# yuanwu2017/llm-d

Hardware: AMD Instinct MI355X
Metric: output tok/s per decode GPU + p50 TTFT, Llama-3-70B P/D-disagg on 8×MI355X (higher is better)
Workload: dtype bf16; 1 GPU; model=Llama-3-70B, global_batch=64, seq_len=5000, isl=5000, osl=250, parallelism=dp1, block_size=64, graphs=True, kv_cache_dtype=auto, async_scheduling=True, setup_prompts_landed=63

## Files before the change

### llmd_amd/csrc/ops/bindings.cpp

```cpp
#include <torch/extension.h>
#include <c10/hip/HIPGuard.h>
#include <c10/hip/HIPStream.h>
#include <hip/hip_runtime.h>
#include <pybind11/stl.h>

#include <map>
#include <mutex>
#include <memory>
#include <vector>

extern "C" {
void llmd_rms_norm(void*, int64_t, const void*, int64_t, const void*, int, int, float, hipStream_t);
void llmd_layer_norm(void*, int64_t, void*, int64_t, void*, int64_t, const void*, const void*, int, int, float,
                     hipStream_t);
void llmd_fused_add_rms_norm(void*, int64_t, void*, int64_t, const void*, int, int, float,
                             hipStream_t);
int llmd_qk_rms_norm(void*, int64_t, const void*, const void*, int, int, int, int, float, hipStream_t);
void llmd_rope_cache(void*, int64_t, const int64_t*, const float*, int, int, int, int,
                     const int64_t*, void*, void*, int64_t, int, int, int, int, float, float, hipStream_t);
void llmd_gated_act(void*, int64_t, const void*, int64_t, int, int, int, float, float, hipStream_t);
int llmd_paged_decode(const void*, int64_t, const void*, const void*, int64_t, int, const int*, int,
                      const int*, int, int, int, int, float, int, const float*, int, int, void*,
                      int64_t, float*, float*, int, float, float, const int*, const int*, const int*,
                      const int*, int, int, int, const int*, hipStream_t);
// ... 28 lines not shown
                        hipStream_t);
int llmd_lora_bgmv(const void*, int64_t, const void*, const void*, int, int, int, int, const int*, float*, void*,
                   int64_t, hipStream_t);
int llmd_skinny_gemm(const void*, int64_t, const void*, int64_t, int, int, int, int, int, int, void*, int64_t,
                     float*, hipStream_t);
int llmd_dgemm_supported(int, int, int);
int llmd_mgemm(const void*, int64_t, const void*, int64_t, int, int, int, int, int, int, void*, int64_t, float*,
               int*, hipStream_t);
int llmd_mgemm_lds(int, int, int);
int llmd_mgemm_partials(const void*, int64_t, const void*, int64_t, int, int, int, int, int, int, float*, hipStream_t);
int llmd_reduce_rope_cache(const float*, int, int, void*, int64_t, const int64_t*, const float*, int, int, int, int,
                           const int64_t*, void*, void*, int64_t, int, int, int, int, float, float, hipStream_t);
int llmd_mgemm_add_rmsnorm(const void*, int64_t, const void*, int64_t, int, int, int, int, int, int, float*, void*,
                           int64_t, const void*, float, void*, int64_t, hipStream_t);
int llmd_mgemm_silu(const void*, int64_t, const void*, int64_t, int, int, int, int, int, void*, int64_t, hipStream_t);
int llmd_pgemm(const void*, int64_t, const void*, int64_t, void*, int64_t, int, int, int, int, int, void*,
               hipStream_t);
int64_t llmd_pgemm_ws_bytes(int, int, int, int, int);
int llmd_pgemm_fp8(const void*, int64_t, const float*, const void*, int64_t, const float*, void*, int64_t, int, int,
                   int, int, void*, hipStream_t);
int64_t llmd_pgemm_fp8_ws_bytes(int, int, int, int);
int llmd_mgemm_fp8(const void*, int64_t, const float*, const void*, int64_t, const float*, int, int, int, int, int,
                   int, void*, int64_t, float*, int*, hipStream_t);
int llmd_vmm_granularity(int, size_t*);
int llmd_vmm_alloc(int, size_t, int, void**, uint64_t*);
int llmd_vmm_export_fd(uint64_t, int*);
int llmd_vmm_import(const int*, int, size_t, int, void**, uint64_t*);
int llmd_vmm_free(void*, size_t, int, const uint64_t*);
int llmd_kvx_handle_size();
int llmd_kvx_dma_blocks(void*, const void*, int64_t, int64_t, const int*, int, int64_t, hipStream_t);
void llmd_moe_topk(const float*, int, int, int, int, const float*, int, int, int, float, int*, float*,
                   hipStream_t);
void llmd_moe_align(const int*, int, int, int, int*, int*, int*, int, int*, int*, hipStream_t);
// ... 428 lines not shown
  CHECK_CUDA(x); CHECK_BF16(x); CHECK_BF16(w); CHECK_BF16(out); CHECK_BF16(residual); CHECK_BF16(gamma);
  CHECK_INNER(x); CHECK_INNER(w); CHECK_INNER(out); CHECK_INNER(residual); CHECK_DT(part, at::kFloat);
  TORCH_CHECK(x.dim() == 2 && w.dim() == 2 && out.dim() == 2 && residual.dim() == 2, "mgemm_add_rmsnorm: 2-D operands");
  const int M = x.size(0), K = x.size(1), N = w.size(0);
  TORCH_CHECK(M >= 1 && M <= 128 && w.size(1) == K && K % 64 == 0 && N % 8 == 0, "mgemm_add_rmsnorm: shapes");
  TORCH_CHECK(out.size(0) == M && out.size(1) == N && residual.size(0) == M && residual.size(1) == N &&
              gamma.numel() == N, "mgemm_add_rmsnorm: output / residual / gamma shape");
  TORCH_CHECK(nsplit > 1 && part.numel() >= nsplit * (int64_t)M * N, "mgemm_add_rmsnorm: split-K workspace");
  int rc = llmd_mgemm_add_rmsnorm(x.data_ptr(), x.stride(0), w.data_ptr(), w.stride(0), M, N, K, (int)wrb,
                                  (int)nsplit, (int)stages, part.data_ptr<float>(), residual.data_ptr(),
                                  residual.stride(0), gamma.data_ptr(), (float)eps, out.data_ptr(), out.stride(0),
                                  cur_stream());
  TORCH_CHECK(rc == 0, "mgemm_add_rmsnorm failed: ", rc);
}

void pgemm(torch::Tensor y, torch::Tensor x, torch::Tensor w, int64_t epi, int64_t variant, bool split_k) {
  const c10::hip::OptionalHIPGuard device_guard(dev_of(y));
  CHECK_CUDA(x); CHECK_BF16(x); CHECK_BF16(w); CHECK_BF16(y); CHECK_INNER(x); CHECK_INNER(w); CHECK_INNER(y);
  TORCH_CHECK(x.dim() == 2 && w.dim() == 2 && y.dim() == 2, "pgemm: 2-D operands");
  const int64_t M = x.size(0), K = x.size(1), N = w.size(0);
  TORCH_CHECK(w.size(1) == K && K % 64 == 0 && N % 256 == 0, "pgemm: N % 256 == 0, K % 64 == 0");
  TORCH_CHECK(y.size(0) == M && y.size(1) == ((epi == 1 || epi == 3) ? N / 2 : N), "pgemm: output shape");
  TORCH_CHECK(epi != 3 || (variant >= 3 && variant <= 6), "pgemm: epi 3 (SiLU on the [gate; up] weight) needs variant 3-6");
  TORCH_CHECK(x.stride(0) % 8 == 0 && w.stride(0) % 8 == 0 && y.stride(0) % 8 == 0, "pgemm: 16-B row alignment");
  torch::Tensor ws;
  const int64_t wsb = split_k ? llmd_pgemm_ws_bytes((int)M, (int)N, (int)K, (int)epi, (int)variant) : 0;
  if (wsb > 0) ws = torch::empty({wsb / 4}, x.options().dtype(torch::kFloat));
  int rc = llmd_pgemm(x.data_ptr(), x.stride(0), w.data_ptr(), w.stride(0), y.data_ptr(), y.stride(0), (int)M,
                      (int)N, (int)K, (int)epi, (int)variant, wsb > 0 ? ws.data_ptr() : nullptr, cur_stream());
  TORCH_CHECK(rc == 0, "pgemm failed: ", rc);
}

void pgemm_fp8(torch::Tensor y, torch::Tensor xq, torch::Tensor xs, torch::Tensor wq, torch::Tensor ws, int64_t epi,
               bool split_k) {
  const c10::hip::OptionalHIPGuard device_guard(dev_of(y));
  CHECK_CUDA(xq); CHECK_BF16(y); CHECK_INNER(xq); CHECK_INNER(wq); CHECK_INNER(y);
  TORCH_CHECK(xq.scalar_type() == at::kFloat8_e4m3fn && wq.scalar_type() == at::kFloat8_e4m3fn, "pgemm_fp8: e4m3fn");
  TORCH_CHECK(xs.scalar_type() == at::kFloat && ws.scalar_type() == at::kFloat, "pgemm_fp8: fp32 scales");
  TORCH_CHECK(xs.is_contiguous() && ws.is_contiguous(), "pgemm_fp8: contiguous scales");
  TORCH_CHECK(xq.dim() == 2 && wq.dim() == 2 && y.dim() == 2, "pgemm_fp8: 2-D operands");
  const int64_t M = xq.size(0), K = xq.size(1), N = wq.size(0);
  TORCH_CHECK(wq.size(1) == K && K % 128 == 0 && N % 256 == 0, "pgemm_fp8: N % 256 == 0, K % 128 == 0");
  TORCH_CHECK(xs.numel() == M && ws.numel() == N, "pgemm_fp8: per-token / per-channel scales");
  TORCH_CHECK(epi == 0 || epi == 3, "pgemm_fp8: epi 0 or 3");
  TORCH_CHECK(y.size(0) == M && y.size(1) == (epi == 3 ? N / 2 : N), "pgemm_fp8: output shape");
// ... 740 lines not shown
  m.def("kvx_dma_blocks", &kvx_dma_blocks);
  m.def("kvx_ipc_export", &kvx_ipc_export);
  m.def("kvx_ipc_open", &kvx_ipc_open);
  m.def("kvx_ipc_close", &kvx_ipc_close);
  m.def("mla_attention", &mla_attention);
  m.def("mla_v2_shape", &mla_v2_shape, "H=128 MLA kernel shape: 10 * waves + head blocks per wave");
  m.def("skinny_gemm", &skinny_gemm);
  m.def("skinny_supported", &skinny_supported);
  m.def("mgemm", &mgemm);
  m.def("mgemm_partials", &mgemm_partials, "split-K partials of the medium-M GEMM (no reduce); returns nsplit");
  m.def("reduce_rope_cache", &reduce_rope_cache, "QKV split-K reduce + RoPE + paged cache write");
  m.def("mgemm_add_rmsnorm", &mgemm_add_rmsnorm, "decode o / down projection with residual-add + RMSNorm in its split-K reduce");
  m.def("pgemm_fp8", &pgemm_fp8, "prefill fp8 W8A8 GEMM (256x256 LDS-DMA tiles on 16x16x128 f8f6f4 MFMA), "
        "per-token x per-channel scales, optional fused SiLU-and-mul");
  m.def("pgemm", &pgemm, "prefill bf16 GEMM (256x256 LDS-DMA MFMA tiles), optional fused SiLU-and-mul",
        py::arg("y"), py::arg("x"), py::arg("w"), py::arg("epi"), py::arg("variant"), py::arg("split_k") = true);
  m.def("mgemm_fp8", &mgemm_fp8);
  m.def("mgemm_lds", [](int64_t M, int64_t wrb, int64_t stages) { return llmd_mgemm_lds((int)M, (int)wrb, (int)stages); });
  m.def("lora_bgmv", &lora_bgmv);
  m.def("mla_rope_cache", &mla_rope_cache);
  m.def("vmm_granularity", &vmm_granularity);
  m.def("vmm_pool", &vmm_pool);
  m.def("vmm_import", &vmm_import);
  m.def("vmm_release", &vmm_release);
  m.def("moe_topk", &moe_topk);
  m.def("moe_align", &moe_align, py::arg("ids"), py::arg("E"), py::arg("sorted_ids"), py::arg("tile_expert"),
        py::arg("expert_offsets"), py::arg("total_p"), py::arg("inv"), py::arg("tile_m") = 0);
  m.def("moe_gemm", &moe_gemm, py::arg("X"), py::arg("topk"), py::arg("sorted_ids"), py::arg("tile_expert"),
        py::arg("W"), py::arg("Y"), py::arg("mode"), py::arg("act"), py::arg("alpha"), py::arg("limit"),
        py::arg("a_rows_are_slots"), py::arg("bias"), py::arg("tile_m") = 0);
  m.def("moe_combine", &moe_combine);
// ... 33 lines not shown
```

### llmd_amd/csrc/ops/pgemm.hip

```cpp
#include <algorithm>
#include <type_traits>

#include "llmd_common.h"

using namespace llmd;

namespace {

constexpr int BM = 256, BN = 256, BK = 64, NT = 512;
constexpr int HALF = 16384;
constexpr int BUF = 4 * HALF;
constexpr int LDS_BYTES = 2 * BUF;
constexpr int GROUP_M = 8;

enum { EPI_NONE = 0, EPI_SILU = 1, EPI_F32 = 2, EPI_SILU_STD = 3 };

__device__ __forceinline__ void dma16(const void* src, char* lds) {
  __builtin_amdgcn_global_load_lds((const void __attribute__((address_space(1)))*)src,
                                   (void __attribute__((address_space(3)))*)lds, 16, 0, 0);
}

__device__ __forceinline__ void wait_vm(int n) {
  switch (n) {
    case 0: asm volatile("s_waitcnt vmcnt(0)" ::: "memory"); break;
// ... 774 lines not shown
#pragma unroll 4
    for (int it = 0; it < 16; ++it) {
      const int row = wc * 64 + it * 4 + (lane >> 4), c = lane & 15;
      const int m = m0 + wr * 128 + row;
      const int off = row * 256 + ((c ^ (row & 15)) * 16);
      float gf[8], uf[8], of[8];
      unpack8(*reinterpret_cast<const u32x4_t*>(gimg + off), gf);
      unpack8(*reinterpret_cast<const u32x4_t*>(uimg + off), uf);
#pragma unroll
      for (int e = 0; e < 8; ++e) of[e] = gf[e] / (1.f + __expf(-gf[e])) * uf[e];
      if (m < M) *reinterpret_cast<u32x4_t*>(C + (int64_t)m * ldc + n0 / 2 + c * 8) = pack8(of);
    }
  }
}

template <int EPI>
__global__ __launch_bounds__(NT6, 1) void pgemm7_kernel(const uint16_t* __restrict__ A, int64_t lda,
                                                        const uint16_t* __restrict__ W, int64_t ldw,
                                                        uint16_t* __restrict__ C, int64_t ldc, int M, int N, int K,
                                                        int ntiles) {
  constexpr int RB = 37;
  __shared__ __attribute__((aligned(1024))) char lds[2 * BUF6];
  const int tiles_m = (M + BM - 1) / BM, tiles_n = N / BN;
  const int P = gridDim.x;
  const int b = xcd_remap(blockIdx.x, P);
  const int nt = (ntiles - b + P - 1) / P;
  const int nk = K / BK;
  const int S = nt * nk;

  const int tid = threadIdx.x, lane = tid & 63;
// ... 197 lines not shown
__host__ inline void pgemm_plan(int M, int N, int K, int epi, int& full, int& tail, int& nsplit) {
  const int ntiles = ((M + BM - 1) / BM) * (N / BN), nk = K / BK;
  full = ntiles;
  tail = 0;
  nsplit = 1;
  const int t = ntiles % PG_CUS;
  if (epi != EPI_NONE || t == 0 || 2 * t > PG_CUS || nk < 32) return;
  int s = PG_CUS / t;
  s = std::min(s, nk / 8);
  if (s < 2) return;
  full = ntiles - t;
  tail = t;
  nsplit = s;
}

}

extern "C" int64_t llmd_pgemm_ws_bytes(int M, int N, int K, int epi, int variant) {
  if (M <= 0 || N % BN || K % BK) return 0;
  int full, tail, nsplit;
  pgemm_plan(M, N, K, epi, full, tail, nsplit);
  return nsplit > 1 ? (int64_t)nsplit * tail * BM * BN * 4 : 0;
}

extern "C" int llmd_pgemm(const void* A, int64_t lda, const void* W, int64_t ldw, void* C, int64_t ldc, int M, int N,
                          int K, int epi, int variant, void* ws, hipStream_t st) {
  if (M <= 0) return 0;
  if (N % BN || K % BK || lda % 8 || ldw % 8 || ldc % 8) return -1;
  if (epi == EPI_SILU_STD && (variant < 3 || variant > 6)) return -3;
  if ((int64_t)(M - 1) * lda + K > 0x7fffffffLL || (int64_t)(N - 1) * ldw + K > 0x7fffffffLL) return -2;
  const int ntiles = ((M + BM - 1) / BM) * (N / BN);
  if (variant == 6) {
    if (((int64_t)(M - 1) * lda + K) * 2 > 0x7fffffffLL || ((int64_t)(N - 1) * ldw + K) * 2 > 0x7fffffffLL) return -2;
    int full = ntiles, tail = 0, nsplit = 1;
    if (ws != nullptr) pgemm_plan(M, N, K, epi == EPI_SILU_STD ? EPI_SILU : epi, full, tail, nsplit);
    const auto* a = (const uint16_t*)A;
    const auto* w = (const uint16_t*)W;
    auto* c = (uint16_t*)C;
    const int P = std::min(full, PG_CUS);
    if (epi == EPI_SILU_STD)
      hipLaunchKernelGGL(pgemm7_kernel<EPI_SILU_STD>, dim3(P), dim3(NT6), 0, st, a, lda, w, ldw, c, ldc, M, N, K, full);
    else if (epi == EPI_NONE && full > 0)
      hipLaunchKernelGGL(pgemm7_kernel<EPI_NONE>, dim3(P), dim3(NT6), 0, st, a, lda, w, ldw, c, ldc, M, N, K, full);
    else if (epi != EPI_NONE)
      return -3;
    if (nsplit > 1) {
      hipLaunchKernelGGL((pgemm6_kernel<EPI_F32, 37, 0>), dim3(tail * nsplit), dim3(NT6), 0, st, a, lda, w, ldw, c, ldc,
                         M, N, K, full, nsplit, (float*)ws);
      hipLaunchKernelGGL(pgemm_splitk_reduce, dim3(tail * (BM / 8)), dim3(256), 0, st, (const float*)ws, nsplit,
                         tail, full, c, ldc, M, N);
    }
    return (int)hipGetLastError();
  }
  if (variant >= 3 && variant <= 5) {
    if (((int64_t)(M - 1) * lda + K) * 2 > 0x7fffffffLL || ((int64_t)(N - 1) * ldw + K) * 2 > 0x7fffffffLL) return -2;
    int full = ntiles, tail = 0, nsplit = 1;
    if (ws != nullptr) pgemm_plan(M, N, K, epi, full, tail, nsplit);
    const auto* a = (const uint16_t*)A;
    const auto* w = (const uint16_t*)W;
    auto* c = (uint16_t*)C;
    auto launch = [&](auto k_silu, auto k_std, auto k_none, auto k_f32) {
      if (epi == EPI_SILU)
        hipLaunchKernelGGL(k_silu, dim3(full), dim3(NT6), 0, st, a, lda, w, ldw, c, ldc, M, N, K, 0, 1, nullptr);
      else if (epi == EPI_SILU_STD)
        hipLaunchKernelGGL(k_std, dim3(full), dim3(NT6), 0, st, a, lda, w, ldw, c, ldc, M, N, K, 0, 1, nullptr);
      else if (full > 0)
        hipLaunchKernelGGL(k_none, dim3(full), dim3(NT6), 0, st, a, lda, w, ldw, c, ldc, M, N, K, 0, 1, nullptr);
      if (nsplit > 1) {
        hipLaunchKernelGGL(k_f32, dim3(tail * nsplit), dim3(NT6), 0, st, a, lda, w, ldw, c, ldc, M, N, K, full,
                           nsplit, (float*)ws);
        hipLaunchKernelGGL(pgemm_splitk_reduce, dim3(tail * (BM / 8)), dim3(256), 0, st, (const float*)ws, nsplit,
                           tail, full, c, ldc, M, N);
      }
    };
    if (variant == 3)
      launch(pgemm6_kernel<EPI_SILU, 37, 0>, pgemm6_kernel<EPI_SILU_STD, 37, 0>, pgemm6_kernel<EPI_NONE, 37, 0>,
             pgemm6_kernel<EPI_F32, 37, 0>);
    else if (variant == 4)
      launch(pgemm6_kernel<EPI_SILU, 37, 16>, pgemm6_kernel<EPI_SILU_STD, 37, 16>, pgemm6_kernel<EPI_NONE, 37, 16>,
             pgemm6_kernel<EPI_F32, 37, 16>);
    else
      launch(pgemm6_kernel<EPI_SILU, 44, 0>, pgemm6_kernel<EPI_SILU_STD, 44, 0>, pgemm6_kernel<EPI_NONE, 44, 0>,
// ... 63 lines not shown
```

### llmd_amd/models/llama.py

```python
from __future__ import annotations

from typing import Optional

import torch

from llmd_amd import ops
from llmd_amd.engine.attn_meta import AttnMeta
from llmd_amd.engine.config import ModelConfig
from llmd_amd.parallel.state import get_state

from .layers import ColumnLinear, LMHead, PagedAttention, RMSNorm, RowLinear, VocabEmbedding, wants_fp8_input


class LlamaMLP(torch.nn.Module):
    def __init__(self, cfg: ModelConfig, device):
        super().__init__()
        self.gate_up = ColumnLinear(cfg.hidden_size, 2 * cfg.intermediate_size, device=device)
        self.down = RowLinear(cfg.intermediate_size, cfg.hidden_size, device=device)

    def forward(self, x):
        return self.down(self.hidden(x))

    def hidden(self, x):
        gu = self.gate_up
        if (gu.lora is None and gu.bias is None and not wants_fp8_input(self.down) and x.dim() == 2
                and gu.weight.dtype == torch.bfloat16):
            v = ops.pgemm_silu_plan(x, gu.weight)
            if v is not None:
                return ops.pgemm_silu(x, gu.weight, variant=v)
            p = ops.mgemm_silu_plan(x, gu.weight)
            if p is not None:
                return ops.mgemm_silu(x, gu.weight, p)
        x0 = x[0] if isinstance(x, tuple) else x
        if (wants_fp8_input(self.down) and wants_fp8_input(gu) and gu.bias is None and x0.dim() == 2
                and ops._gpu(x0) and ops.pgemm8_silu_planned(x0.shape[0], gu.weight.shape[0], gu.weight.shape[1])):
            xq, xs = x if isinstance(x, tuple) else ops.quant_fp8_rows(x)
            if ops.pgemm_fp8_ok(xq, gu.weight):
                return ops.quant_fp8_rows(ops.pgemm_fp8(xq, xs, gu.weight, gu.weight_scale, epi=3))
        h = gu(x)
        if wants_fp8_input(self.down):
            return ops.gated_act_quant(h, ops.ACT_SILU)
        return ops.gated_act(h, ops.ACT_SILU)


# ... 172 lines not shown
```

### llmd_amd/ops/__init__.py

```python
from __future__ import annotations

import logging
import math
import os
from typing import Optional

import torch

from . import reference as ref

log = logging.getLogger("llmd.ops")

_C = None
_C_ERR: Exception | None = None


def native():
    global _C, _C_ERR
    if _C is not None:
        return _C
    import importlib

    debug = os.environ.get("LLMD_KERNEL_DEBUG", "0") == "1"
    name = "llmd_amd._C_debug" if debug else "llmd_amd._C"
# ... 1087 lines not shown


def mgemm_ok(x: torch.Tensor, w: torch.Tensor, max_m: int = 256) -> bool:
    M = x.shape[0] if x.dim() == 2 else -1
    return (_gpu(x) and 1 <= M <= max_m and x.shape[1] % 64 == 0 and x.dtype == torch.bfloat16
            and w.dtype == torch.bfloat16 and w.shape[0] % 4 == 0 and x.stride(-1) == 1 and x.stride(0) % 8 == 0
            and w.is_contiguous())


_MGEMM_MS = (64, 96, 128, 192, 256)


PGEMM_VARIANT = int(os.environ.get("LLMD_PGEMM_VARIANT", "0"))


def pgemm(x: torch.Tensor, w: torch.Tensor, epi: int = 0, out: Optional[torch.Tensor] = None,
          variant: Optional[int] = None, split_k: bool = True) -> torch.Tensor:
    M = x.shape[0]
    N = w.shape[0]
    if out is None:
        out = torch.empty(M, N // 2 if epi in (1, 3) else N, dtype=x.dtype, device=x.device)
    native().pgemm(out, x, w, epi, PGEMM_VARIANT if variant is None else variant, split_k)
    return out


def pgemm_silu(x: torch.Tensor, w: torch.Tensor, variant: int = 3, out: Optional[torch.Tensor] = None):
    return pgemm(x, w, epi=3, out=out, variant=variant, split_k=False)


def pgemm_pack_gate_up(w: torch.Tensor) -> torch.Tensor:
    F2, K = w.shape
    F = F2 // 2
    assert F % 128 == 0, F
    g = w[:F].view(F // 128, 128, K)
    u = w[F:].view(F // 128, 128, K)
    return torch.stack((g, u), 1).reshape(F2, K).contiguous()


def pgemm_ok(x: torch.Tensor, w: torch.Tensor) -> bool:
    return (x.dim() == 2 and x.dtype == torch.bfloat16 and w.dtype == torch.bfloat16 and x.is_cuda
            and w.shape[0] % 256 == 0 and w.shape[1] % 64 == 0 and x.stride(-1) == 1 and x.stride(0) % 8 == 0
            and w.is_contiguous())
# ... 13 lines not shown
PGEMM_MIN_M = int(os.environ.get("LLMD_PGEMM_MIN_M", "256"))
_pgemm_pick: dict = {}


def _time_ms(fn, reps: int = 2) -> float:
    fn()
    st, en = torch.cuda.Event(enable_timing=True), torch.cuda.Event(enable_timing=True)
    st.record()
    for _ in range(reps):
        fn()
    en.record()
    en.synchronize()
    return st.elapsed_time(en) / reps


def pgemm_plan(M: int, N: int, K: int) -> Optional[tuple[int, bool]]:
    from .pgemm_table import PGEMM_TABLE

    e = PGEMM_TABLE.get(((M + 255) // 256, N, K))
    return None if e is None else e[0]


def pgemm_silu_plan(x: torch.Tensor, w: torch.Tensor) -> Optional[int]:
    if PGEMM_AUTO == "0" or x.shape[0] < PGEMM_MIN_M or not pgemm_ok(x, w) or (w.shape[0] // 2) % 128:
        return None
    from .pgemm_table import PGEMM_TABLE

    e = PGEMM_TABLE.get(("silu", (x.shape[0] + 255) // 256, w.shape[0], w.shape[1]))
    return None if e is None or e[0] is None else e[0][0]


def pgemm_wins(x: torch.Tensor, w: torch.Tensor) -> Optional[tuple[int, bool]]:
    M, (N, K) = x.shape[0], w.shape
    if PGEMM_AUTO != "measure":
        return pgemm_plan(M, N, K)
    key = ((M + 255) // 256, N, K)
    c = _pgemm_pick.get(key, False)
    if c is False:
        if torch.cuda.is_current_stream_capturing():
            return None
        y = torch.empty(M, N, dtype=x.dtype, device=x.device)
        t_pg = _time_ms(lambda: pgemm(x, w, out=y))
        t_bl = _time_ms(lambda: torch.nn.functional.linear(x, w))
        c = _pgemm_pick[key] = (PGEMM_VARIANT, True) if t_pg < 0.97 * t_bl else None
        msg = (f"prefill GEMM M~{M} N={N} K={K}: pgemm {t_pg:.3f} ms, hipBLASLt {t_bl:.3f} ms -> "
               f"{'pgemm' if c else 'hipBLASLt'}")
        log.debug(msg)
        if os.environ.get("LLMD_PGEMM_VERBOSE") == "1":
            import sys

            print(msg, file=sys.stderr, flush=True)
    return c


def linear(x: torch.Tensor, w: torch.Tensor, bias: Optional[torch.Tensor] = None) -> torch.Tensor:
    if PGEMM_AUTO != "0" and x.dim() == 2 and x.shape[0] >= PGEMM_MIN_M and pgemm_ok(x, w):
        plan = pgemm_wins(x, w)
        if plan is not None:
            y = pgemm(x, w, variant=plan[0], split_k=plan[1])
            return y if bias is None else y.add_(bias)
    if _SKINNY:
        M = x.shape[0] if x.dim() == 2 else 0
        if 33 <= M <= 256 and mgemm_ok(x, w):
            plan = mgemm_choice(M, w.shape[0], w.shape[1])
            if plan is not None:
                y = mgemm(x, w, plan)
                return y if bias is None else y.add_(bias)
        if skinny_ok(x, w):
            plan = dgemm_choice(M, w.shape[0], w.shape[1])
            if plan is not None:
                y = skinny_gemm(x, w, plan)
                return y if bias is None else y.add_(bias)
    return torch.nn.functional.linear(x, w, bias)

# ... 3 lines not shown
```

### llmd_amd/ops/pgemm_table.py

```python

PGEMM_TABLE = {
    (2, 4096, 4096): (None, 35.5, 26.0),
    (3, 4096, 4096): (None, 38.8, 28.9),
    (4, 4096, 4096): (None, 44.9, 34.1),
    (6, 4096, 4096): (None, 57.2, 46.9),
    (8, 4096, 4096): (None, 67.2, 57.4),
    (12, 4096, 4096): (None, 78.7, 75.7),
    (16, 4096, 4096): (None, 92.9, 88.1),
    (18, 4096, 4096): ((3, True), 127.5, 141.3),
    (20, 4096, 4096): (None, 137.7, 135.1),
    (24, 4096, 4096): (None, 159.1, 153.9),
    (32, 4096, 4096): (None, 183.7, 175.9),
    (2, 4096, 14336): ((3, True), 65.4, 78.2),
    (3, 4096, 14336): ((3, True), 84.4, 93.0),
    (4, 4096, 14336): ((3, True), 101.4, 112.2),
    (6, 4096, 14336): (None, 152.1, 151.7),
    (8, 4096, 14336): ((3, True), 172.0, 182.4),
    (12, 4096, 14336): (None, 258.8, 246.9),
    (16, 4096, 14336): (None, 318.4, 290.9),
    (18, 4096, 14336): ((0, True), 405.5, 756.1),
    (20, 4096, 14336): (None, 455.5, 443.1),
    (24, 4096, 14336): (None, 528.7, 506.9),
    (32, 4096, 14336): (None, 678.8, 595.5),
    (2, 5120, 8192): ((3, True), 54.1, 57.0),
# ... 8 lines not shown
    (24, 5120, 8192): (None, 339.1, 328.3),
    (32, 5120, 8192): ((3, False), 486.1, 651.4),
    (2, 6144, 4096): (None, 40.4, 31.8),
    (3, 6144, 4096): (None, 47.3, 34.3),
    (4, 6144, 4096): (None, 56.4, 45.6),
    (6, 6144, 4096): (None, 71.4, 61.0),
    (8, 6144, 4096): (None, 77.7, 73.3),
    (12, 6144, 4096): ((3, True), 127.1, 138.1),
    (16, 6144, 4096): (None, 157.6, 151.7),
    (18, 6144, 4096): (None, 167.5, 165.3),
    (20, 6144, 4096): (None, 178.9, 174.3),
    (24, 6144, 4096): (None, 225.7, 227.6),
    (32, 6144, 4096): (None, 273.4, 264.5),
    (2, 8192, 4096): (None, 46.6, 35.9),
    (3, 8192, 4096): (None, 56.6, 42.0),
    (4, 8192, 4096): (None, 66.0, 55.9),
    (6, 8192, 4096): (None, 78.3, 75.4),
    (8, 8192, 4096): (None, 92.7, 88.8),
    (12, 8192, 4096): (None, 156.9, 150.5),
    (16, 8192, 4096): (None, 183.5, 177.8),
    (18, 8192, 4096): (None, 227.5, 226.9),
    (20, 8192, 4096): ((3, True), 248.7, 354.7),
    (24, 8192, 4096): (None, 275.3, 264.3),
    (32, 8192, 4096): (None, 365.5, 349.5),
    (2, 8192, 8192): (None, 69.3, 68.2),
    (3, 8192, 8192): (None, 92.9, 78.5),
    (4, 8192, 8192): (None, 107.0, 105.9),
    (6, 8192, 8192): (None, 148.4, 143.4),
    (8, 8192, 8192): (None, 174.9, 170.3),
    (12, 8192, 8192): (None, 301.9, 291.4),
    (16, 8192, 8192): (None, 350.5, 336.4),
    (18, 8192, 8192): (None, 436.4, 440.9),
    (20, 8192, 8192): ((3, False), 482.5, 667.5),
    (24, 8192, 8192): (None, 523.1, 506.2),
    (32, 8192, 8192): (None, 701.3, 675.2),
    (2, 8192, 14336): (None, 112.9, 116.2),
    (3, 8192, 14336): (None, 173.8, 143.9),
    (4, 8192, 14336): ((3, True), 192.9, 206.2),
    (6, 8192, 14336): (None, 267.5, 258.3),
    (8, 8192, 14336): (None, 325.4, 307.1),
    (12, 8192, 14336): (None, 523.5, 525.7),
    (16, 8192, 14336): (None, 630.5, 600.7),
    (18, 8192, 14336): (None, 781.4, 801.0),
    (20, 8192, 14336): ((3, True), 856.5, 1081.4),
    (24, 8192, 14336): (None, 1012.4, 909.5),
    (32, 8192, 14336): (None, 1342.3, 1210.8),
    (2, 8192, 28672): ((3, True), 212.5, 314.7),
    (3, 8192, 28672): (None, 335.0, 270.3),
    (4, 8192, 28672): (None, 364.2, 362.3),
    (6, 8192, 28672): (None, 583.4, 508.3),
    (8, 8192, 28672): (None, 653.8, 628.6),
    (12, 8192, 28672): ((3, True), 1004.7, 1044.5),
    (16, 8192, 28672): (None, 1316.1, 1238.6),
    (18, 8192, 28672): (None, 1549.3, 1591.1),
    (20, 8192, 28672): ((3, True), 1694.7, 2340.8),
    (24, 8192, 28672): (None, 1998.6, 1912.4),
    (32, 8192, 28672): (None, 2659.9, 2518.2),
    (2, 10240, 8192): (None, 81.1, 80.3),
    (3, 10240, 8192): (None, 102.3, 102.1),
    (4, 10240, 8192): (None, 135.7, 127.8),
    (6, 10240, 8192): (None, 167.0, 164.9),
    (8, 10240, 8192): ((3, True), 249.0, 263.2),
    (12, 10240, 8192): (None, 341.3, 325.5),
    (16, 10240, 8192): ((3, True), 466.9, 667.1),
    (18, 10240, 8192): (None, 529.0, 492.6),
    (20, 10240, 8192): ((3, True), 597.1, 665.1),
    (24, 10240, 8192): (None, 691.7, 659.0),
    (32, 10240, 8192): (None, 879.8, 853.7),
    (2, 28672, 4096): (None, 89.8, 88.7),
    ("silu", 2, 28672, 4096): ((6, False), 91.3, 103.9),
    (3, 28672, 4096): (None, 152.1, 134.0),
    ("silu", 3, 28672, 4096): (None, 163.8, 150.6),
    (4, 28672, 4096): (None, 178.2, 172.4),
    ("silu", 4, 28672, 4096): ((3, False), 182.7, 192.4),
    (6, 28672, 4096): (None, 262.4, 257.7),
    ("silu", 6, 28672, 4096): ((6, False), 272.9, 288.6),
    (8, 28672, 4096): (None, 353.9, 332.9),
    ("silu", 8, 28672, 4096): ((6, False), 362.4, 374.1),
    (12, 28672, 4096): (None, 516.7, 520.9),
    ("silu", 12, 28672, 4096): ((6, False), 537.0, 566.1),
    (16, 28672, 4096): (None, 648.9, 611.8),
    ("silu", 16, 28672, 4096): ((6, False), 669.8, 692.7),
    (18, 28672, 4096): (None, 746.3, 701.2),
    ("silu", 18, 28672, 4096): ((6, False), 755.3, 786.9),
    (20, 28672, 4096): ((3, True), 831.7, 893.4),
    ("silu", 20, 28672, 4096): ((3, False), 852.6, 976.0),
    (24, 28672, 4096): ((3, True), 1008.1, 1076.1),
    ("silu", 24, 28672, 4096): ((6, False), 1028.2, 1180.9),
    (32, 28672, 4096): (None, 1288.0, 1251.4),
    ("silu", 32, 28672, 4096): ((3, False), 1323.5, 1389.5),
    (2, 28672, 8192): (None, 197.6, 186.2),
    ("silu", 2, 28672, 8192): (None, 201.1, 200.1),
    (3, 28672, 8192): (None, 274.2, 261.6),
    ("silu", 3, 28672, 8192): (None, 318.8, 273.5),
    (4, 28672, 8192): (None, 347.3, 340.0),
    ("silu", 4, 28672, 8192): ((3, False), 355.7, 417.4),
    (6, 28672, 8192): (None, 511.5, 512.9),
    ("silu", 6, 28672, 8192): ((3, False), 526.5, 536.0),
    (8, 28672, 8192): (None, 660.7, 660.7),
    ("silu", 8, 28672, 8192): (None, 691.6, 687.8),
    (12, 28672, 8192): (None, 975.6, 974.7),
    ("silu", 12, 28672, 8192): (None, 1047.4, 1020.5),
    (16, 28672, 8192): (None, 1241.5, 1209.7),
    ("silu", 16, 28672, 8192): (None, 1278.9, 1270.3),
    (18, 28672, 8192): (None, 1511.8, 1412.0),
    ("silu", 18, 28672, 8192): (None, 1484.1, 1469.4),
    (20, 28672, 8192): ((3, False), 1601.0, 1652.6),
    ("silu", 20, 28672, 8192): ((3, False), 1636.7, 1722.6),
    (24, 28672, 8192): ((3, True), 1940.4, 2082.5),
    ("silu", 24, 28672, 8192): ((3, False), 1981.2, 2163.8),
    (32, 28672, 8192): (None, 2464.3, 2435.3),
    ("silu", 32, 28672, 8192): (None, 2552.3, 2566.0),
    (2, 57344, 8192): (None, 384.7, 371.3),
    ("silu", 2, 57344, 8192): (None, 393.1, 388.1),
    (3, 57344, 8192): (None, 528.2, 522.0),
# ... 21 lines not shown
```

Before: 383.3 output tok/s (whole job).

## Add half-height tail tiles to prefill GEMM to balance the last wave

Adds a new prefill GEMM tail mode that runs the leftover tiles of a partial wave as two 128-row half-tiles each, so more CUs stay busy when the tile count leaves a small remainder modulo the CU count. It plumbs a tail-form argument through the C ABI, bindings and Python wrappers, and adds a host-side plan query. The per-shape table is updated to select the half-tile form for several Llama-relevant shapes, including the gate_up SiLU path at some M buckets. Half tiles cost more weight traffic per output element and add a second kernel launch.

```diff
diff --git a/llmd_amd/csrc/ops/bindings.cpp b/llmd_amd/csrc/ops/bindings.cpp
--- a/llmd_amd/csrc/ops/bindings.cpp
+++ b/llmd_amd/csrc/ops/bindings.cpp
@@ -66,9 +66,10 @@
 int llmd_mgemm_add_rmsnorm(const void*, int64_t, const void*, int64_t, int, int, int, int, int, int, float*, void*,
                            int64_t, const void*, float, void*, int64_t, hipStream_t);
 int llmd_mgemm_silu(const void*, int64_t, const void*, int64_t, int, int, int, int, int, void*, int64_t, hipStream_t);
-int llmd_pgemm(const void*, int64_t, const void*, int64_t, void*, int64_t, int, int, int, int, int, void*,
+int llmd_pgemm(const void*, int64_t, const void*, int64_t, void*, int64_t, int, int, int, int, int, int, void*,
                hipStream_t);
-int64_t llmd_pgemm_ws_bytes(int, int, int, int, int);
+int64_t llmd_pgemm_ws_bytes(int, int, int, int, int, int);
+int llmd_pgemm_plan(int, int, int, int, int, int*, int*, int*);
 int llmd_pgemm_fp8(const void*, int64_t, const float*, const void*, int64_t, const float*, void*, int64_t, int, int,
                    int, int, void*, hipStream_t);
 int64_t llmd_pgemm_fp8_ws_bytes(int, int, int, int);
@@ -527,7 +528,7 @@
   TORCH_CHECK(rc == 0, "mgemm_add_rmsnorm failed: ", rc);
 }
 
-void pgemm(torch::Tensor y, torch::Tensor x, torch::Tensor w, int64_t epi, int64_t variant, bool split_k) {
+void pgemm(torch::Tensor y, torch::Tensor x, torch::Tensor w, int64_t epi, int64_t variant, int64_t tail) {
   const c10::hip::OptionalHIPGuard device_guard(dev_of(y));
   CHECK_CUDA(x); CHECK_BF16(x); CHECK_BF16(w); CHECK_BF16(y); CHECK_INNER(x); CHECK_INNER(w); CHECK_INNER(y);
   TORCH_CHECK(x.dim() == 2 && w.dim() == 2 && y.dim() == 2, "pgemm: 2-D operands");
@@ -537,11 +538,21 @@
   TORCH_CHECK(epi != 3 || (variant >= 3 && variant <= 6), "pgemm: epi 3 (SiLU on the [gate; up] weight) needs variant 3-6");
   TORCH_CHECK(x.stride(0) % 8 == 0 && w.stride(0) % 8 == 0 && y.stride(0) % 8 == 0, "pgemm: 16-B row alignment");
   torch::Tensor ws;
-  const int64_t wsb = split_k ? llmd_pgemm_ws_bytes((int)M, (int)N, (int)K, (int)epi, (int)variant) : 0;
+  TORCH_CHECK(tail >= 0 && tail <= 2, "pgemm: tail 0 (none), 1 (split-K) or 2 (half tiles)");
+  TORCH_CHECK(tail != 2 || variant == 3, "pgemm: the half-tile tail needs variant 3");
+  const int64_t wsb = llmd_pgemm_ws_bytes((int)M, (int)N, (int)K, (int)epi, (int)variant, (int)tail);
   if (wsb > 0) ws = torch::empty({wsb / 4}, x.options().dtype(torch::kFloat));
   int rc = llmd_pgemm(x.data_ptr(), x.stride(0), w.data_ptr(), w.stride(0), y.data_ptr(), y.stride(0), (int)M,
-                      (int)N, (int)K, (int)epi, (int)variant, wsb > 0 ? ws.data_ptr() : nullptr, cur_stream());
+                      (int)N, (int)K, (int)epi, (int)variant, (int)tail, wsb > 0 ? ws.data_ptr() : nullptr,
+                      cur_stream());
   TORCH_CHECK(rc == 0, "pgemm failed: ", rc);
+}
+
+std::tuple<int64_t, int64_t, int64_t, int64_t, int64_t> pgemm_plan(int64_t M, int64_t N, int64_t K, int64_t epi,
+                                                                   int64_t tail) {
+  int full = 0, t = 0, nsplit = 1;
+  const int form = llmd_pgemm_plan((int)M, (int)N, (int)K, (int)epi, (int)tail, &full, &t, &nsplit);
+  return {form, full, t, nsplit, llmd_pgemm_ws_bytes((int)M, (int)N, (int)K, (int)epi, 3, (int)tail)};
 }
 
 void pgemm_fp8(torch::Tensor y, torch::Tensor xq, torch::Tensor xs, torch::Tensor wq, torch::Tensor ws, int64_t epi,
@@ -1312,7 +1323,8 @@
   m.def("pgemm_fp8", &pgemm_fp8, "prefill fp8 W8A8 GEMM (256x256 LDS-DMA tiles on 16x16x128 f8f6f4 MFMA), "
         "per-token x per-channel scales, optional fused SiLU-and-mul");
   m.def("pgemm", &pgemm, "prefill bf16 GEMM (256x256 LDS-DMA MFMA tiles), optional fused SiLU-and-mul",
-        py::arg("y"), py::arg("x"), py::arg("w"), py::arg("epi"), py::arg("variant"), py::arg("split_k") = true);
+        py::arg("y"), py::arg("x"), py::arg("w"), py::arg("epi"), py::arg("variant"), py::arg("tail") = 1);
+  m.def("pgemm_plan", &pgemm_plan, "launch plan of the prefill GEMM under a tail form (host only)");
   m.def("mgemm_fp8", &mgemm_fp8);
   m.def("mgemm_lds", [](int64_t M, int64_t wrb, int64_t stages) { return llmd_mgemm_lds((int)M, (int)wrb, (int)stages); });
   m.def("lora_bgmv", &lora_bgmv);
diff --git a/llmd_amd/csrc/ops/pgemm.hip b/llmd_amd/csrc/ops/pgemm.hip
--- a/llmd_amd/csrc/ops/pgemm.hip
+++ b/llmd_amd/csrc/ops/pgemm.hip
@@ -812,6 +812,178 @@
   }
 }
 
+constexpr int HM = 128;
+constexpr int IMGH = 16384;
+
+template <int EPI>
+__global__ __launch_bounds__(NT6, 1) void pgemm6h_kernel(const uint16_t* __restrict__ A, int64_t lda,
+                                                         const uint16_t* __restrict__ W, int64_t ldw,
+                                                         uint16_t* __restrict__ C, int64_t ldc, int M, int N, int K,
+                                                         int tile0) {
+  static_assert(EPI == EPI_NONE || EPI == EPI_SILU_STD, "half tiles: no packed-SiLU or fp32-partial form");
+  __shared__ __attribute__((aligned(1024))) char lds[2 * BUF6];
+  const int tiles_m = (M + BM - 1) / BM, tiles_n = N / BN;
+  const int b = xcd_remap(blockIdx.x, gridDim.x);
+  const int nk = K / BK;
+  int tm, tn;
+  tile_mn(tile0 + (b >> 1), tiles_m, tiles_n, tm, tn);
+  const int m0 = tm * BM + (b & 1) * HM, n0 = tn * BN;
+  if (m0 >= M) return;
+
+  const int tid = threadIdx.x, lane = tid & 63;
+  const int w = __builtin_amdgcn_readfirstlane(tid >> 6);
+  const int wr = w >> 1, wc = w & 1;
+
+  const __amdgpu_buffer_rsrc_t ra = __builtin_amdgcn_make_buffer_rsrc((void*)A, 0, 0x7fffffff, 0x00020000);
+  const __amdgpu_buffer_rsrc_t rw = __builtin_amdgcn_make_buffer_rsrc((void*)W, 0, 0x7fffffff, 0x00020000);
+  uint32_t va[4], vw[8];
+#pragma unroll
+  for (int j = 0; j < 4; ++j) {
+    const int row = 32 * w + 8 * j + (lane >> 3);
+    const int c = (lane & 7) ^ ((row >> 1) & 7);
+    va[j] = m0 + row < M ? (uint32_t)(((m0 + row) * lda + c * 8) * 2) : 0x80000000u;
+  }
+#pragma unroll
+  for (int j = 0; j < 8; ++j) {
+    const int row = 64 * w + 8 * j + (lane >> 3);
+    const int c = (lane & 7) ^ ((row >> 1) & 7);
+    const int wrow = EPI == EPI_SILU_STD ? (row < 128 ? 0 : N / 2 - 128) + tn * 128 + row : n0 + row;
+    vw[j] = (uint32_t)((wrow * ldw + c * 8) * 2);
+  }
+  auto dma_a = [&](int kt, int j) {
+    const uint32_t so = (uint32_t)(min(kt, nk - 1) * BK * 2);
+    char* dst = lds + (kt & 1) * BUF6 + (4 * w + j) * 1024;
+    __builtin_amdgcn_raw_ptr_buffer_load_lds(ra, (__attribute__((address_space(3))) void*)dst, 16, va[j], so, 0, 0);
+  };
+  auto dma_w = [&](int kt, int j) {
+    const uint32_t so = (uint32_t)(min(kt, nk - 1) * BK * 2);
+    char* dst = lds + (kt & 1) * BUF6 + OPB6 + (8 * w + j) * 1024;
+    __builtin_amdgcn_raw_ptr_buffer_load_lds(rw, (__attribute__((address_space(3))) void*)dst, 16, vw[j], so, 0, 0);
+  };
+
+  const int fr = lane & 15, fq = lane >> 4;
+  const int rd0 = fr * 128 + ((fq ^ ((fr >> 1) & 7)) * 16);
+  const int rd1 = fr * 128 + (((4 + fq) ^ ((fr >> 1) & 7)) * 16);
+  const int a_rd = (wr * 64) * 128, w_rd = OPB6 + (wc * 128) * 128;
+
+  f32x4_t acc[4][8];
+#pragma unroll
+  for (int i = 0; i < 4; ++i)
+#pragma unroll
+    for (int j = 0; j < 8; ++j) acc[i][j] = f32x4_t{0.f, 0.f, 0.f, 0.f};
+  s16x8_t fa0[4], fw0[8], fa1[4], fw1[8];
+
+#pragma unroll
+  for (int j = 0; j < 4; ++j) dma_a(0, j);
+#pragma unroll
+  for (int j = 0; j < 8; ++j) dma_w(0, j);
+#pragma unroll
+  for (int j = 0; j < 4; ++j) dma_a(1, j);
+#pragma unroll
+  for (int j = 0; j < 8; ++j) dma_w(1, j);
+  asm volatile("s_waitcnt vmcnt(12)" ::: "memory");
+  bar();
+  fa0[0] = *reinterpret_cast<const s16x8_t*>(lds + a_rd + rd0);
+  __builtin_amdgcn_sched_barrier(0);
+#pragma unroll
+  for (int i = 0; i < 8; ++i) {
+    fw0[i] = *reinterpret_cast<const s16x8_t*>(lds + w_rd + i * 2048 + rd0);
+    __builtin_amdgcn_sched_barrier(0);
+  }
+#pragma unroll
+  for (int i = 1; i < 4; ++i) {
+    fa0[i] = *reinterpret_cast<const s16x8_t*>(lds + a_rd + i * 2048 + rd0);
+    __builtin_amdgcn_sched_barrier(0);
+  }
+  __builtin_amdgcn_s_waitcnt(0xC07F);
+  __builtin_amdgcn_sched_barrier(0);
+  asm volatile("s_nop 4" ::: "memory");
+  __builtin_amdgcn_sched_barrier(0);
+
+  for (int kt = 0; kt < nk; ++kt) {
+    const char* cur = lds + (kt & 1) * BUF6;
+    const char* nxt = lds + ((kt & 1) ^ 1) * BUF6;
+#pragma unroll
+    for (int t = 0; t < 32; ++t) {
+      const int i = t >> 3, j = t & 7;
+      if (t <= 8) __builtin_amdgcn_s_waitcnt(0xC07F | (10 << 8));
+      mfma16_acc(acc[i][j], fw0[j], fa0[i]);
+      if (t == 0) {
+        fa1[0] = *reinterpret_cast<const s16x8_t*>(cur + a_rd + rd1);
+      } else if (t < 9) {
+        fw1[t - 1] = *reinterpret_cast<const s16x8_t*>(cur + w_rd + (t - 1) * 2048 + rd1);
+      } else if (t < 12) {
+        fa1[t - 8] = *reinterpret_cast<const s16x8_t*>(cur + a_rd + (t - 8) * 2048 + rd1);
+      } else if (t == 20) {
+        __builtin_amdgcn_s_waitcnt(0xC07F);
+        bar();
+      } else if (t > 20 && (t - 21) % 3 == 0) {
+        dma_a(kt + 2, (t - 21) / 3);
+      }
+      __builtin_amdgcn_sched_barrier(0);
+    }
+#pragma unroll
+    for (int t = 0; t < 32; ++t) {
+      const int i = t >> 3, j = t & 7;
+      mfma16_acc(acc[i][j], fw1[j], fa1[i]);
+      if (t < 16 && t % 2 == 0) {
+        dma_w(kt + 2, t / 2);
+      } else if (t == 16) {
+        asm volatile("s_waitcnt vmcnt(12)" ::: "memory");
+        bar();
+      } else if (t == 17) {
+        fa0[0] = *reinterpret_cast<const s16x8_t*>(nxt + a_rd + rd0);
+      } else if (t > 17 && t < 26) {
+        fw0[t - 18] = *reinterpret_cast<const s16x8_t*>(nxt + w_rd + (t - 18) * 2048 + rd0);
+      } else if (t >= 26 && t < 29) {
+        fa0[t - 25] = *reinterpret_cast<const s16x8_t*>(nxt + a_rd + (t - 25) * 2048 + rd0);
+      }
+      __builtin_amdgcn_sched_barrier(0);
+    }
+  }
+  mfma_drain();
+  __builtin_amdgcn_sched_barrier(0);
+  asm volatile("s_waitcnt vmcnt(0) lgkmcnt(0)" ::: "memory");
+  __syncthreads();
+  char* img = lds + w * IMGH;
+#pragma unroll
+  for (int i = 0; i < 4; ++i)
+#pragma unroll
+    for (int j = 0; j < 8; ++j) {
+      const int row = 16 * i + fr, col = 16 * j + 4 * fq;
+      const f32x4_t v = acc[i][j];
+      u32x2_t p;
+      p[0] = (uint32_t)f2bf(v[0]) | ((uint32_t)f2bf(v[1]) << 16);
+      p[1] = (uint32_t)f2bf(v[2]) | ((uint32_t)f2bf(v[3]) << 16);
+      *reinterpret_cast<u32x2_t*>(img + row * 256 + (((col >> 3) ^ (row & 15)) * 16) + (col & 7) * 2) = p;
+    }
+  __syncthreads();
+  if constexpr (EPI == EPI_NONE) {
+#pragma unroll 4
+    for (int it = 0; it < 16; ++it) {
+      const int row = it * 4 + (lane >> 4), c = lane & 15;
+      const int m = m0 + wr * 64 + row;
+      const u32x4_t v = *reinterpret_cast<const u32x4_t*>(img + row * 256 + ((c ^ (row & 15)) * 16));
+      if (m < M) *reinterpret_cast<u32x4_t*>(C + (int64_t)m * ldc + n0 + wc * 128 + c * 8) = v;
+    }
+  } else {
+    const char* gimg = lds + (wr * 2) * IMGH;
+    const char* uimg = gimg + IMGH;
+#pragma unroll 4
+    for (int it = 0; it < 8; ++it) {
+      const int row = wc * 32 + it * 4 + (lane >> 4), c = lane & 15;
+      const int m = m0 + wr * 64 + row;
+      const int off = row * 256 + ((c ^ (row & 15)) * 16);
+      float gf[8], uf[8], of[8];
+      unpack8(*reinterpret_cast<const u32x4_t*>(gimg + off), gf);
+      unpack8(*reinterpret_cast<const u32x4_t*>(uimg + off), uf);
+#pragma unroll
+      for (int e = 0; e < 8; ++e) of[e] = gf[e] / (1.f + __expf(-gf[e])) * uf[e];
+      if (m < M) *reinterpret_cast<u32x4_t*>(C + (int64_t)m * ldc + n0 / 2 + c * 8) = pack8(of);
+    }
+  }
+}
+
 template <int EPI>
 __global__ __launch_bounds__(NT6, 1) void pgemm7_kernel(const uint16_t* __restrict__ A, int64_t lda,
                                                         const uint16_t* __restrict__ W, int64_t ldw,
@@ -1039,20 +1211,49 @@
   nsplit = s;
 }
 
-}
-
-extern "C" int64_t llmd_pgemm_ws_bytes(int M, int N, int K, int epi, int variant) {
-  if (M <= 0 || N % BN || K % BK) return 0;
+enum { TAIL_NONE = 0, TAIL_SPLITK = 1, TAIL_HALF = 2 };
+
+__host__ inline bool pgemm_half_plan(int M, int N, int epi, int& full, int& tail) {
+  const int ntiles = ((M + BM - 1) / BM) * (N / BN);
+  full = ntiles;
+  tail = 0;
+  const int t = ntiles % PG_CUS;
+  if ((epi != EPI_NONE && epi != EPI_SILU_STD) || t == 0 || 2 * t > PG_CUS) return false;
+  full = ntiles - t;
+  tail = t;
+  return true;
+}
+
+}
+
+extern "C" int llmd_pgemm_plan(int M, int N, int K, int epi, int tail_form, int* full, int* tail, int* nsplit) {
+  *full = *tail = 0;
+  *nsplit = 1;
+  if (M <= 0 || N % BN || K % BK) return TAIL_NONE;
+  *full = ((M + BM - 1) / BM) * (N / BN);
+  if (tail_form == TAIL_SPLITK) {
+    pgemm_plan(M, N, K, epi, *full, *tail, *nsplit);
+    return *nsplit > 1 ? TAIL_SPLITK : TAIL_NONE;
+  }
+  if (tail_form == TAIL_HALF) return pgemm_half_plan(M, N, epi, *full, *tail) ? TAIL_HALF : TAIL_NONE;
+  return TAIL_NONE;
+}
+
+extern "C" int64_t llmd_pgemm_ws_bytes(int M, int N, int K, int epi, int variant, int tail_form) {
+  if (M <= 0 || N % BN || K % BK || tail_form != TAIL_SPLITK) return 0;
   int full, tail, nsplit;
   pgemm_plan(M, N, K, epi, full, tail, nsplit);
   return nsplit > 1 ? (int64_t)nsplit * tail * BM * BN * 4 : 0;
 }
 
 extern "C" int llmd_pgemm(const void* A, int64_t lda, const void* W, int64_t ldw, void* C, int64_t ldc, int M, int N,
-                          int K, int epi, int variant, void* ws, hipStream_t st) {
+                          int K, int epi, int variant, int tail_form, void* ws, hipStream_t st) {
   if (M <= 0) return 0;
   if (N % BN || K % BK || lda % 8 || ldw % 8 || ldc % 8) return -1;
   if (epi == EPI_SILU_STD && (variant < 3 || variant > 6)) return -3;
+  if (tail_form < TAIL_NONE || tail_form > TAIL_HALF) return -3;
+  if (tail_form == TAIL_HALF && variant != 3) return -3;
+  if (tail_form != TAIL_SPLITK) ws = nullptr;
   if ((int64_t)(M - 1) * lda + K > 0x7fffffffLL || (int64_t)(N - 1) * ldw + K > 0x7fffffffLL) return -2;
   const int ntiles = ((M + BM - 1) / BM) * (N / BN);
   if (variant == 6) {
@@ -1081,16 +1282,25 @@
     if (((int64_t)(M - 1) * lda + K) * 2 > 0x7fffffffLL || ((int64_t)(N - 1) * ldw + K) * 2 > 0x7fffffffLL) return -2;
     int full = ntiles, tail = 0, nsplit = 1;
     if (ws != nullptr) pgemm_plan(M, N, K, epi, full, tail, nsplit);
+    const bool half = tail_form == TAIL_HALF && pgemm_half_plan(M, N, epi, full, tail);
     const auto* a = (const uint16_t*)A;
     const auto* w = (const uint16_t*)W;
     auto* c = (uint16_t*)C;
     auto launch = [&](auto k_silu, auto k_std, auto k_none, auto k_f32) {
       if (epi == EPI_SILU)
         hipLaunchKernelGGL(k_silu, dim3(full), dim3(NT6), 0, st, a, lda, w, ldw, c, ldc, M, N, K, 0, 1, nullptr);
-      else if (epi == EPI_SILU_STD)
+      else if (epi == EPI_SILU_STD && full > 0)
         hipLaunchKernelGGL(k_std, dim3(full), dim3(NT6), 0, st, a, lda, w, ldw, c, ldc, M, N, K, 0, 1, nullptr);
-      else if (full > 0)
+      else if (epi != EPI_SILU_STD && full > 0)
         hipLaunchKernelGGL(k_none, dim3(full), dim3(NT6), 0, st, a, lda, w, ldw, c, ldc, M, N, K, 0, 1, nullptr);
+      if (half) {
+        if (epi == EPI_SILU_STD)
+          hipLaunchKernelGGL(pgemm6h_kernel<EPI_SILU_STD>, dim3(2 * tail), dim3(NT6), 0, st, a, lda, w, ldw, c, ldc,
+                             M, N, K, full);
+        else
+          hipLaunchKernelGGL(pgemm6h_kernel<EPI_NONE>, dim3(2 * tail), dim3(NT6), 0, st, a, lda, w, ldw, c, ldc, M,
+                             N, K, full);
+      }
       if (nsplit > 1) {
         hipLaunchKernelGGL(k_f32, dim3(tail * nsplit), dim3(NT6), 0, st, a, lda, w, ldw, c, ldc, M, N, K, full,
                            nsplit, (float*)ws);
diff --git a/llmd_amd/models/llama.py b/llmd_amd/models/llama.py
--- a/llmd_amd/models/llama.py
+++ b/llmd_amd/models/llama.py
@@ -25,9 +25,9 @@
         gu = self.gate_up
         if (gu.lora is None and gu.bias is None and not wants_fp8_input(self.down) and x.dim() == 2
                 and gu.weight.dtype == torch.bfloat16):
-            v = ops.pgemm_silu_plan(x, gu.weight)
-            if v is not None:
-                return ops.pgemm_silu(x, gu.weight, variant=v)
+            p = ops.pgemm_silu_plan(x, gu.weight)
+            if p is not None:
+                return ops.pgemm_silu(x, gu.weight, variant=p[0], tail=p[1])
             p = ops.mgemm_silu_plan(x, gu.weight)
             if p is not None:
                 return ops.mgemm_silu(x, gu.weight, p)
diff --git a/llmd_amd/ops/__init__.py b/llmd_amd/ops/__init__.py
--- a/llmd_amd/ops/__init__.py
+++ b/llmd_amd/ops/__init__.py
@@ -1125,18 +1125,23 @@
 PGEMM_VARIANT = int(os.environ.get("LLMD_PGEMM_VARIANT", "0"))
 
 
+PGEMM_TAILS = {False: 0, True: 1, "half": 2}
+
+
 def pgemm(x: torch.Tensor, w: torch.Tensor, epi: int = 0, out: Optional[torch.Tensor] = None,
-          variant: Optional[int] = None, split_k: bool = True) -> torch.Tensor:
+          variant: Optional[int] = None, split_k: bool = True, tail=None) -> torch.Tensor:
     M = x.shape[0]
     N = w.shape[0]
     if out is None:
         out = torch.empty(M, N // 2 if epi in (1, 3) else N, dtype=x.dtype, device=x.device)
-    native().pgemm(out, x, w, epi, PGEMM_VARIANT if variant is None else variant, split_k)
+    native().pgemm(out, x, w, epi, PGEMM_VARIANT if variant is None else variant,
+                   PGEMM_TAILS[bool(split_k) if tail is None else tail])
     return out
 
 
-def pgemm_silu(x: torch.Tensor, w: torch.Tensor, variant: int = 3, out: Optional[torch.Tensor] = None):
-    return pgemm(x, w, epi=3, out=out, variant=variant, split_k=False)
+def pgemm_silu(x: torch.Tensor, w: torch.Tensor, variant: int = 3, out: Optional[torch.Tensor] = None,
+               tail=False):
+    return pgemm(x, w, epi=3, out=out, variant=variant, tail=tail)
 
 
 def pgemm_pack_gate_up(w: torch.Tensor) -> torch.Tensor:
@@ -1180,23 +1185,23 @@
     return st.elapsed_time(en) / reps
 
 
-def pgemm_plan(M: int, N: int, K: int) -> Optional[tuple[int, bool]]:
+def pgemm_plan(M: int, N: int, K: int) -> Optional[tuple]:
     from .pgemm_table import PGEMM_TABLE
 
     e = PGEMM_TABLE.get(((M + 255) // 256, N, K))
     return None if e is None else e[0]
 
 
-def pgemm_silu_plan(x: torch.Tensor, w: torch.Tensor) -> Optional[int]:
+def pgemm_silu_plan(x: torch.Tensor, w: torch.Tensor) -> Optional[tuple]:
     if PGEMM_AUTO == "0" or x.shape[0] < PGEMM_MIN_M or not pgemm_ok(x, w) or (w.shape[0] // 2) % 128:
         return None
     from .pgemm_table import PGEMM_TABLE
 
     e = PGEMM_TABLE.get(("silu", (x.shape[0] + 255) // 256, w.shape[0], w.shape[1]))
-    return None if e is None or e[0] is None else e[0][0]
-
-
-def pgemm_wins(x: torch.Tensor, w: torch.Tensor) -> Optional[tuple[int, bool]]:
+    return None if e is None else e[0]
+
+
+def pgemm_wins(x: torch.Tensor, w: torch.Tensor) -> Optional[tuple]:
     M, (N, K) = x.shape[0], w.shape
     if PGEMM_AUTO != "measure":
         return pgemm_plan(M, N, K)
@@ -1223,7 +1228,7 @@
     if PGEMM_AUTO != "0" and x.dim() == 2 and x.shape[0] >= PGEMM_MIN_M and pgemm_ok(x, w):
         plan = pgemm_wins(x, w)
         if plan is not None:
-            y = pgemm(x, w, variant=plan[0], split_k=plan[1])
+            y = pgemm(x, w, variant=plan[0], tail=plan[1])
             return y if bias is None else y.add_(bias)
     if _SKINNY:
         M = x.shape[0] if x.dim() == 2 else 0
diff --git a/llmd_amd/ops/pgemm_table.py b/llmd_amd/ops/pgemm_table.py
--- a/llmd_amd/ops/pgemm_table.py
+++ b/llmd_amd/ops/pgemm_table.py
@@ -4,7 +4,7 @@
     (3, 4096, 4096): (None, 38.8, 28.9),
     (4, 4096, 4096): (None, 44.9, 34.1),
     (6, 4096, 4096): (None, 57.2, 46.9),
-    (8, 4096, 4096): (None, 67.2, 57.4),
+    (8, 4096, 4096): ((3, 'half'), 53.4, 55.2),
     (12, 4096, 4096): (None, 78.7, 75.7),
     (16, 4096, 4096): (None, 92.9, 88.1),
     (18, 4096, 4096): ((3, True), 127.5, 141.3),
@@ -46,7 +46,7 @@
     (32, 6144, 4096): (None, 273.4, 264.5),
     (2, 8192, 4096): (None, 46.6, 35.9),
     (3, 8192, 4096): (None, 56.6, 42.0),
-    (4, 8192, 4096): (None, 66.0, 55.9),
+    (4, 8192, 4096): ((3, 'half'), 50.8, 55.4),
     (6, 8192, 4096): (None, 78.3, 75.4),
     (8, 8192, 4096): (None, 92.7, 88.8),
     (12, 8192, 4096): (None, 156.9, 150.5),
@@ -57,13 +57,13 @@
     (32, 8192, 4096): (None, 365.5, 349.5),
     (2, 8192, 8192): (None, 69.3, 68.2),
     (3, 8192, 8192): (None, 92.9, 78.5),
-    (4, 8192, 8192): (None, 107.0, 105.9),
+    (4, 8192, 8192): ((3, 'half'), 95.0, 104.5),
     (6, 8192, 8192): (None, 148.4, 143.4),
     (8, 8192, 8192): (None, 174.9, 170.3),
     (12, 8192, 8192): (None, 301.9, 291.4),
     (16, 8192, 8192): (None, 350.5, 336.4),
     (18, 8192, 8192): (None, 436.4, 440.9),
-    (20, 8192, 8192): ((3, False), 482.5, 667.5),
+    (20, 8192, 8192): ((3, 'half'), 458.1, 670.9),
     (24, 8192, 8192): (None, 523.1, 506.2),
     (32, 8192, 8192): (None, 701.3, 675.2),
     (2, 8192, 14336): (None, 112.9, 116.2),
@@ -89,7 +89,7 @@
     (24, 8192, 28672): (None, 1998.6, 1912.4),
     (32, 8192, 28672): (None, 2659.9, 2518.2),
     (2, 10240, 8192): (None, 81.1, 80.3),
-    (3, 10240, 8192): (None, 102.3, 102.1),
+    (3, 10240, 8192): ((3, 'half'), 89.5, 99.0),
     (4, 10240, 8192): (None, 135.7, 127.8),
     (6, 10240, 8192): (None, 167.0, 164.9),
     (8, 10240, 8192): ((3, True), 249.0, 263.2),
@@ -102,7 +102,7 @@
     (2, 28672, 4096): (None, 89.8, 88.7),
     ("silu", 2, 28672, 4096): ((6, False), 91.3, 103.9),
     (3, 28672, 4096): (None, 152.1, 134.0),
-    ("silu", 3, 28672, 4096): (None, 163.8, 150.6),
+    ("silu", 3, 28672, 4096): ((3, 'half'), 139.7, 145.6),
     (4, 28672, 4096): (None, 178.2, 172.4),
     ("silu", 4, 28672, 4096): ((3, False), 182.7, 192.4),
     (6, 28672, 4096): (None, 262.4, 257.7),
@@ -130,7 +130,7 @@
     (6, 28672, 8192): (None, 511.5, 512.9),
     ("silu", 6, 28672, 8192): ((3, False), 526.5, 536.0),
     (8, 28672, 8192): (None, 660.7, 660.7),
-    ("silu", 8, 28672, 8192): (None, 691.6, 687.8),
+    ("silu", 8, 28672, 8192): ((3, 'half'), 647.0, 682.0),
     (12, 28672, 8192): (None, 975.6, 974.7),
     ("silu", 12, 28672, 8192): (None, 1047.4, 1020.5),
     (16, 28672, 8192): (None, 1241.5, 1209.7),
```

New measurement: 384.5 output tok/s (whole job) (median of 6 runs). No clear change (+0.3%).
